# zju3dv/neuralbody

Measured on AMD Instinct MI355X. Metric: ray_samples_per_sec, higher is better.
Workload: dtype f16+f6/f4

## Files before the change

### neuralbody_amd/csrc/nb_march_fold.hip

```cpp
#include "nb_f6_ops.h"
#include "nb_march_hooks.h"

using namespace nbm;

namespace {

#ifndef NB_FP4_TERMS
#define NB_FP4_TERMS 3
#endif
constexpr bool FP4_K[2] = {(NB_FP4_TERMS & 1) != 0, (NB_FP4_TERMS & 2) != 0};
constexpr bool ANY_FP4 = FP4_K[0] || FP4_K[1];
constexpr int TERM_ORDER[2] = {(FP4_K[0] && !FP4_K[1]) ? 1 : 0, (FP4_K[0] && !FP4_K[1]) ? 0 : 1};
__host__ __device__ constexpr int term_pieces(int k) { return FP4_K[k] ? 1 : 2; }
__host__ __device__ constexpr int block_pieces(int mt) { return (4 * mt + mt * term_pieces(0) + mt * term_pieces(1) + 1) & ~1; }
__host__ __device__ constexpr int cross_piece(int mt, int slot, int m) {
    return 4 * mt + (slot == 0 ? 0 : mt * term_pieces(TERM_ORDER[0])) + m * term_pieces(TERM_ORDER[slot]);
}
constexpr int S_R = 8;
__host__ __device__ constexpr int phase_pieces(int nb, int mt) { return nb * block_pieces(mt); }
constexpr int N_PH = 4;
constexpr int PH_NB[N_PH] = {4, 4, 4, 2};
constexpr int PH_MT[N_PH] = {2, 2, 1, 1};
__host__ __device__ constexpr int phase_p0(int ph) {
    int p = 0;
// ... 365 lines not shown
    xhi = red_max16i(xhi); yhi = red_max16i(yhi); zhi = red_max16i(zhi);
    const int any = __builtin_amdgcn_ballot_w64(take) != 0ull;
    if (write && os == 0) {
        i32x4 *d = reinterpret_cast<i32x4 *>(actz + WBOX_OFF + (wslot * 4 + part) * 32);
        d[0] = i32x4{xlo, ylo, zlo, xhi};
        d[1] = i32x4{yhi, zhi, any, 0};
    }
}

struct Prep {
    int xlo, ylo, zlo, nx, nxy, n, k0;
    int K;
    int tier;
    int any;
};
__device__ __forceinline__ int box_count(int xlo, int ylo, int zlo, int xhi, int yhi, int zhi) {
    return (xhi < xlo || yhi < ylo || zhi < zlo) ? 0 : (xhi - xlo + 1) * (yhi - ylo + 1) * (zhi - zlo + 1);
}
template <int NW>
__device__ __forceinline__ Prep prep_wg(const char *actz, int part) {
    int xlo = BOX_BIG, ylo = BOX_BIG, zlo = BOX_BIG, xhi = -1, yhi = -1, zhi = -1;
    int n16[NW], any = 0;
#pragma unroll
    for (int w = 0; w < NW; ++w) {
        const i32x4 *s = reinterpret_cast<const i32x4 *>(actz + WBOX_OFF + (w * 4 + part) * 32);
        const i32x4 a = s[0], b = s[1];
        any |= b.z;
        n16[w] = box_count(a.x, a.y, a.z, a.w, b.x, b.y);
        xlo = min(xlo, a.x); ylo = min(ylo, a.y); zlo = min(zlo, a.z);
        xhi = max(xhi, a.w); yhi = max(yhi, b.x); zhi = max(zhi, b.y);
    }
    Prep p;
    p.xlo = xlo; p.ylo = ylo; p.zlo = zlo;
    p.nx = xhi - xlo + 1;
    p.nxy = p.nx * (yhi - ylo + 1);
    p.n = box_count(xlo, ylo, zlo, xhi, yhi, zhi);
    const int n0 = __builtin_amdgcn_readlane(p.n, 0), n1 = __builtin_amdgcn_readlane(p.n, 16), n2 = __builtin_amdgcn_readlane(p.n, 32),
              n3 = __builtin_amdgcn_readlane(p.n, 48);
    p.K = n0 + n1 + n2 + n3;
    p.k0 = part == 0 ? 0 : (part == 1 ? n0 : (part == 2 ? n0 + n1 : n0 + n1 + n2));
    p.tier = 0;
    p.any = any;
    if constexpr (NW > 1) {
        if (p.K > K_CAP && p.K <= KM_CAP) {
            p.tier = 3;
        } else if (p.K > K_CAP) {
            int worst = 0;
#pragma unroll
            for (int w = 0; w < NW; ++w)
                worst = max(worst, __builtin_amdgcn_readlane(n16[w], 0) + __builtin_amdgcn_readlane(n16[w], 16) +
                                       __builtin_amdgcn_readlane(n16[w], 32) + __builtin_amdgcn_readlane(n16[w], 48));
            p.tier = worst <= K_CAP ? 1 : 2;
        }
    }
    return p;
}

struct TblLoad {
    int rid[2], idx[2];
};
__device__ __forceinline__ TblLoad tbl_issue(const Prep &p, const Lvl &lv, int wave, int os) {
    TblLoad t;
    const float rcp_xy = __builtin_amdgcn_rcpf((float)max(p.nxy, 1)), rcp_x = __builtin_amdgcn_rcpf((float)max(p.nx, 1));
#pragma unroll
    for (int q = 0; q < 2; ++q) {
        const int j = 64 * q + 16 * wave + os;
        t.rid[q] = -1;
        t.idx[q] = -1;
        if (j < p.n) {
            const int vz = (int)(((float)j + 0.5f) * rcp_xy);
            const int r = mad24(vz, -p.nxy, j);
            const int vy = (int)(((float)r + 0.5f) * rcp_x);
            const int vx = mad24(vy, -p.nx, r);
            const int lin = mad24(mad24(p.zlo + vz, lv.H, p.ylo + vy), lv.W, p.xlo + vx);
            t.rid[q] = lv.grid[lin];
            t.idx[q] = p.k0 + j;
        }
    }
    return t;
}
__device__ __forceinline__ void tbl_store(char *actz, const TblLoad &t, const Lvl &lv, unsigned zero_off, int K, int tid) {
    unsigned *tbl = reinterpret_cast<unsigned *>(actz + TBL_OFF);
#pragma unroll
    for (int q = 0; q < 2; ++q)
        if (t.idx[q] >= 0) tbl[t.idx[q]] = t.rid[q] < 0 ? zero_off : (unsigned)(lv.rbase + t.rid[q]) << 10;
    if (tid < 16 && K + tid < ((K + 15) & ~15)) tbl[K + tid] = zero_off;
}
__device__ __forceinline__ void tbl_pass(char *actz, unsigned zero_off, int k_lo, int K, int tid) {
    if (tid >= K_CAP) return;
    unsigned *tbl = reinterpret_cast<unsigned *>(actz + TBL_OFF);
    const int k = k_lo + tid;
    unsigned e = zero_off;
    if (k < K) {
        const int k1 = *reinterpret_cast<const int *>(actz + LVL_OFF + 1 * 32 + 20), k2 = *reinterpret_cast<const int *>(actz + LVL_OFF + 2 * 32 + 20),
                  k3 = *reinterpret_cast<const int *>(actz + LVL_OFF + 3 * 32 + 20);
        const int L = (k >= k1) + (k >= k2) + (k >= k3);
        const i32x4 *lp = reinterpret_cast<const i32x4 *>(actz + LVL_OFF + L * 32);
        const i32x4 b0 = lp[0], b1 = lp[1];
        const Lvl lv = load_lvl(actz, L);
        const int j = k - b1.y;
        const float rcp_xy = __builtin_amdgcn_rcpf((float)max(b1.x, 1)), rcp_x = __builtin_amdgcn_rcpf((float)max(b0.w, 1));
        const int vz = (int)(((float)j + 0.5f) * rcp_xy);
        const int r = mad24(vz, -b1.x, j);
        const int vy = (int)(((float)r + 0.5f) * rcp_x);
        const int vx = mad24(vy, -b0.w, r);
        const int lin = mad24(mad24(b0.z + vz, lv.H, b0.y + vy), lv.W, b0.x + vx);
        const int rid = lv.grid[lin];
        if (rid >= 0) e = (unsigned)(lv.rbase + rid) << 10;
    }
    tbl[tid] = e;
}
__device__ __forceinline__ void lvl_store(char *actz, const Prep &p, int tid, int os, int part) {
    if (tid < 64 && os == 0) {
        i32x4 *d = reinterpret_cast<i32x4 *>(actz + LVL_OFF + part * 32);
        d[0] = i32x4{p.xlo, p.ylo, p.zlo, p.nx};
        d[1] = i32x4{p.nxy, p.k0, p.n, 0};
    }
    if (tid == 0) *reinterpret_cast<int *>(actz + HDR_OFF) = p.K;
}

struct UCfg {
    int nch, R;
    unsigned ring;
    int ring_off;
};
__device__ __forceinline__ UCfg ucfg_k(int K, unsigned lds_base, int wave);
__device__ __forceinline__ UCfg ucfg(const char *actz, unsigned lds_base, int wave) {
    return ucfg_k(__builtin_amdgcn_readfirstlane(*reinterpret_cast<const int *>(actz + HDR_OFF)), lds_base, wave);
}
__device__ __forceinline__ UCfg ucfg_k(int K, unsigned lds_base, int wave) {
    UCfg u;
    u.nch = (K + 15) >> 4;
    u.R = u.nch <= 3 ? u.nch : (u.nch == 4 ? 3 : 2);
    u.ring_off = WT_CHUNK * u.nch + wave * u.R * U_CHUNK;
    u.ring = lds_base + (unsigned)u.ring_off;
    return u;
}
__device__ __forceinline__ void dma_chunk(const MarchArgs &a, const char *actz, int lane, int wave, int c, unsigned dst) {
    const int v = ((lane >> 4) << 2) | ((lane >> 1) & 3);
    const unsigned e = *reinterpret_cast<const unsigned *>(actz + TBL_OFF + (16 * c + v) * 4);
    const unsigned voff0 = e + (unsigned)(64 * wave + 16 * ((lane >> 3) & 1) + 8 * (lane & 1)) * 2u;
    const char *base = a.fold.urows;
#pragma unroll
    for (int form = 0; form < 2; ++form)
#pragma unroll
        for (int m = 0; m < 2; ++m) {
            const unsigned voff = voff0 + form * 512 + m * 64;
            const unsigned d = dst + form * 2048 + m * 1024;
            asm volatile(
                "s_mov_b32 m0, %2\n\t"
                "s_nop 0\n\t"
                "global_load_lds_dwordx4 %0, %1"
                :
                : "v"(voff), "s"(base), "s"(d)
                : "memory", "m0");
        }
}
__device__ __forceinline__ void dma_initial(const MarchArgs &a, const char *actz, int lane, int wave, const UCfg &u) {
    for (int c = 0; c < u.R; ++c) dma_chunk(a, actz, lane, wave, c, u.ring + c * U_CHUNK);
}
__device__ __forceinline__ void dma_wait() { asm volatile("s_waitcnt vmcnt(0)" ::: "memory"); }

__device__ __forceinline__ void wt_build(char *actz, const Lvl &lv, const GridCoord &g, bool take, int wave, int os, int part, int nch,
                                         int k_lo = 0) {
    const int nt = wave >> 1, n = 16 * (wave & 1) + os;
    {
        char *z = actz + (part >> 1) * 2048 + nt * 1024 + ((part & 1) * 32 + n) * 16;
        for (int c = 0; c < nch; ++c) *reinterpret_cast<i32x4 *>(z + c * WT_CHUNK) = i32x4{0, 0, 0, 0};
    }
    if (take) {
        const i32x4 *lp = reinterpret_cast<const i32x4 *>(actz + LVL_OFF + part * 32);
        const i32x4 b0 = lp[0], b1 = lp[1];
        const LvlIdx q = level_index(lv, g);
        const float fx = (float)q.x0, fy = (float)q.y0, fz = (float)q.z0;
        const float wx[2] = {(fx + 1.f) - q.ix, q.ix - fx};
        const float wy[2] = {(fy + 1.f) - q.iy, q.iy - fy};
        const float wz[2] = {(fz + 1.f) - q.iz, q.iz - fz};
        const int kbase = b1.y - k_lo + mad24(q.z0 - b0.z, b1.x, mad24(q.y0 - b0.y, b0.w, q.x0 - b0.x));
        const int sbase = nt * 1024 + n * 16;
        float cw[8];
        int ad[8];
#pragma unroll
        for (int corner = 0; corner < 8; ++corner) {
            const int dx = corner & 1, dy = (corner >> 1) & 1, dz = corner >> 2;
            const int xx = q.x0 + dx, yy = q.y0 + dy, zz = q.z0 + dz;
            const bool inb = (unsigned)xx < (unsigned)lv.W && (unsigned)yy < (unsigned)lv.H && (unsigned)zz < (unsigned)lv.D;
            cw[corner] = (wx[dx] * wy[dy]) * wz[dz];
            const int k = kbase + dx + dy * b0.w + dz * b1.x;
            const int off = ((k << 8) & ~0xfff) | ((k << 6) & 0x200) | ((k << 1) & 0xe);
            ad[corner] = (inb && (unsigned)k < (unsigned)(16 * nch)) ? off + sbase : DUMMY_OFF;
        }
#pragma unroll
        for (int cp = 0; cp < 4; ++cp) {
            const unsigned h = cvt_pk_f16(cw[2 * cp], cw[2 * cp + 1]);
            const unsigned l = cvt_pk_f16(rem16<0>(cw[2 * cp], h), rem16<1>(cw[2 * cp + 1], h));
            *reinterpret_cast<unsigned short *>(actz + ad[2 * cp]) = (unsigned short)(h & 0xffffu);
            *reinterpret_cast<unsigned short *>(actz + ad[2 * cp + 1]) = (unsigned short)(h >> 16);
            *reinterpret_cast<unsigned short *>(actz + ad[2 * cp] + 2048) = (unsigned short)(l & 0xffffu);
            *reinterpret_cast<unsigned short *>(actz + ad[2 * cp + 1] + 2048) = (unsigned short)(l >> 16);
        }
    }
}

__device__ __forceinline__ f16x8 tr_frag(const char *p) {
    const s4v a = __builtin_amdgcn_ds_read_tr16_b64_v4i16((lds_s4p)(p));
    const s4v b = __builtin_amdgcn_ds_read_tr16_b64_v4i16((lds_s4p)(p + 256));
    typedef short s8v __attribute__((ext_vector_type(8)));
    return __builtin_bit_cast(f16x8, s8v{a[0], a[1], a[2], a[3], b[0], b[1], b[2], b[3]});
}
struct FoldFrags {
    f16x8 ah[2], al[2];
    i32x4 bh[2], bl[2];
};
__device__ __forceinline__ void fold_wait(int younger) {
    if (younger >= 2) asm volatile("s_waitcnt vmcnt(8)" ::: "memory");
    else if (younger == 1) asm volatile("s_waitcnt vmcnt(4)" ::: "memory");
    else asm volatile("s_waitcnt vmcnt(0)" ::: "memory");
}
__device__ __forceinline__ void fold_read(FoldFrags &f, const char *ub, const char *wtc) {
#pragma unroll
    for (int m = 0; m < 2; ++m) {
        f.ah[m] = tr_frag(ub + m * 1024);
        f.al[m] = tr_frag(ub + 2048 + m * 1024);
    }
#pragma unroll
    for (int n = 0; n < 2; ++n) {
        f.bh[n] = *reinterpret_cast<const i32x4 *>(wtc + n * 1024);
        f.bl[n] = *reinterpret_cast<const i32x4 *>(wtc + 2048 + n * 1024);
    }
}
__device__ __forceinline__ void fold_mma(const FoldFrags &f, f32x16 (&acc)[2][2]) {
#pragma unroll
    for (int p = 0; p < 3; ++p)
#pragma unroll
        for (int m = 0; m < 2; ++m)
#pragma unroll
            for (int n = 0; n < 2; ++n)
                acc[m][n] = __builtin_amdgcn_mfma_f32_32x32x16_f16(p == 2 ? f.al[m] : f.ah[m], __builtin_bit_cast(f16x8, p == 1 ? f.bl[n] : f.bh[n]),
                                                                   acc[m][n], 0, 0, 0);
}
__device__ __forceinline__ void fold_mfma(const MarchArgs &a, char *actz, int lane, int wave, const UCfg &u, f32x16 (&acc)[2][2],
                                          unsigned *tbuf = nullptr) {
    if (u.nch == 0) return;
    FOLD_SUB(17);
    const int l15 = lane & 15, g4 = lane >> 4;
    const int tro = (g4 >> 1) * 512 + (g4 & 1) * 128 + (l15 >> 2) * 32 + (l15 & 3) * 8;
    const char *wt = actz + lane * 16;
    const char *ring = actz + u.ring_off + tro;
    int issued = u.R - 1;
    FoldFrags f0, f1;
    fold_wait(issued);
    FOLD_SUB(18);
    fold_read(f0, ring, wt);
    NB_HOOK_FOLD_FIRST_READ(f0);
    FOLD_SUB(19);
    auto step = [&](FoldFrags &cur, FoldFrags &nxt, int c, int slot) {
        if (c + u.R < u.nch) {
            asm volatile("s_waitcnt lgkmcnt(0)" : "+v"(cur.ah[0]), "+v"(cur.ah[1]), "+v"(cur.al[0]), "+v"(cur.al[1])::"memory");
            dma_chunk(a, actz, lane, wave, c + u.R, u.ring + slot * U_CHUNK);
            issued = c + u.R;
        }
        if (c + 1 < u.nch) {
            const int ns = slot + 1 == u.R ? 0 : slot + 1;
            fold_wait(issued - (c + 1));
            fold_read(nxt, ring + ns * U_CHUNK, wt + (c + 1) * WT_CHUNK);
        }
        fold_mma(cur, acc);
    };
    int slot = 0;
    for (int c = 0; c < u.nch; c += 2) {
        step(f0, f1, c, slot);
        slot = slot + 1 == u.R ? 0 : slot + 1;
        if (c + 1 < u.nch) {
            step(f1, f0, c + 1, slot);
            slot = slot + 1 == u.R ? 0 : slot + 1;
        }
    }
#pragma unroll
    for (int m = 0; m < 2; ++m) asm volatile("" : "+v"(acc[m][0]), "+v"(acc[m][1]));
    FOLD_SUB(20);
    if (tbuf && lane == 0) tbuf[21] = (unsigned)u.nch;
}

struct WeightStore4 {
    float q[4] = {0.f, 0.f, 0.f, 0.f};
    __device__ __forceinline__ void push(const MarchArgs &a, long long ray, int s, int S, int part, bool valid, float w) {
        if ((S & 15) != 0) {
            if (valid && part == 0) a.weights[ray * S + s] = w;
            return;
        }
        const int slot = s & 15;
#pragma unroll
        for (int i = 0; i < 4; ++i)
            if (slot == part * 4 + i) q[i] = w;
        if (slot == 15 && valid)
            *reinterpret_cast<f32x4 *>(a.weights + ray * S + (s - 15) + part * 4) = f32x4{q[0], q[1], q[2], q[3]};
    }
};

__device__ __forceinline__ float head_sum(const char *actz, int off, float bias) {
    const f32x4 p = *reinterpret_cast<const f32x4 *>(actz + off);
    return ((p.x + p.y) + (p.z + p.w)) + bias;
}
__device__ __noinline__ void list_ill_ray(const char *actz, const float *pk, float *ill, int cap, int sample, int part, float z_step, int ray) {
    const float *recf = reinterpret_cast<const float *>(actz + RAY_OFF) + sample * RAY_FLOATS;
    const f32x4 c0 = *reinterpret_cast<const f32x4 *>(recf + 12);
    const float sigma_raw = head_sum(actz, SCR_A + sample * 16, pk[P_AB]);
    const bool hit = ray >= 0 && fabsf(sigma_raw) < NB_ILL_SIGMA && c0.x > NB_ILL_T_MIN;
    if (__builtin_amdgcn_ballot_w64(hit) == 0ull) return;
    int slot = -1;
    if (hit && part == 0) slot = atomicAdd(reinterpret_cast<int *>(ill), 1);
    slot = __builtin_amdgcn_ds_bpermute((sample & 15) << 2, slot);
    if (!hit || slot >= cap) return;
    float *irec = ill + NB_ILL_HEADER_FLOATS + (long long)slot * NB_ILL_RECORD_FLOATS;
    if (part == 0) {
        *reinterpret_cast<f32x4 *>(irec) = f32x4{__int_as_float(ray), c0.x, recf[16], recf[17]};
        *reinterpret_cast<f32x4 *>(irec + 4) = f32x4{z_step, __fmul_rn(1e10f, recf[11]), sigma_raw, 0.f};
    } else {
        const int ch = part - 1;
        irec[8 + ch] = part == 1 ? c0.y : (part == 2 ? c0.z : c0.w);
        irec[12 + ch] = head_sum(actz, SCR_C + (ch * 64 + sample) * 16, pk[P_RB + ch]);
    }
}

__device__ __forceinline__ void composite_step(char *actz, const float *pk, int sample, int part, float z_step, float z_after, bool last,
                                               const MarchArgs &a, long long ray, int sidx, int S, bool valid, WeightStore4 &wstore, bool ins) {
    float *recf = reinterpret_cast<float *>(actz + RAY_OFF) + sample * RAY_FLOATS;
    const f32x4 c0 = *reinterpret_cast<const f32x4 *>(recf + 12);
    const float sigma_raw = ins ? head_sum(actz, SCR_A + sample * 16, pk[P_AB]) : 0.f;
    const float d = last ? 1e10f : __fsub_rn(z_after, z_step);
    const float dist = __fmul_rn(d, recf[11]);
    const float sig = fmaxf(sigma_raw, 0.f);
    const float alpha = 1.f - expf(-sig * dist);
    const float w = alpha * c0.x;
    if (part == 0) {
        const float depth = recf[16], accw = recf[17];
        recf[12] = c0.x * (__fadd_rn(__fsub_rn(1.f, alpha), 1e-10f));
        recf[16] = fmaf(w, z_step, depth);
        recf[17] = accw + w;
    } else {
        const int ch = part - 1;
        const float o = ins ? head_sum(actz, SCR_C + (ch * 64 + sample) * 16, pk[P_RB + ch]) : 0.f;
        const float col = part == 1 ? c0.y : (part == 2 ? c0.z : c0.w);
        recf[12 + part] = fmaf(w, 1.f / (1.f + expf(-o)), col);
    }
    wstore.push(a, ray, sidx, S, part, valid, w);
    if (NB_HOOK_RAW_IS_OUTPUT && a.raw && valid && part == 0) {
        float o3[3];
#pragma unroll
        for (int ch = 0; ch < 3; ++ch) o3[ch] = ins ? head_sum(actz, SCR_C + (ch * 64 + sample) * 16, pk[P_RB + ch]) : 0.f;
        *reinterpret_cast<f32x4 *>(a.raw + (ray * S + sidx) * 4) = f32x4{o3[0], o3[1], o3[2], sigma_raw};
    }
}

__host__ __device__ inline int pe_slot_col(int a, int slot) {
    if (a >= 3 || slot >= 30) return -1;
    if (slot == 0) return 256 + 27 + a;
    if (slot <= 20) {
        const int k = (slot - 1) >> 1, is_cos = (slot - 1) & 1;
        return 256 + 27 + 3 + 6 * k + 3 * is_cos + a;
    }
    if (slot == 21) return 256 + a;
    const int k = (slot - 22) >> 1, is_cos = (slot - 22) & 1;
    return 256 + 3 + 6 * k + 3 * is_cos + a;
}

template <int MODE, bool CULL>
__global__ __launch_bounds__(256, 2) void nb_march_fold_kernel(MarchArgs a, const char *stream) {
    constexpr bool POINTS = MODE != 0, DENSITY_ONLY = MODE == 2;
    static_assert(!(CULL && POINTS), "sample culling is a property of the ray march");
    saturate_fp16_conversions();
    __shared__ __attribute__((aligned(16))) char lds[LDS_BYTES];
    char *act = lds;
    const int tid = threadIdx.x;
    const int lane = threadIdx.x & 63, wave = __builtin_amdgcn_readfirstlane(threadIdx.x >> 6);
    const int grp = xcd_remap(blockIdx.x, a.n_wave_groups);
    long long ray = (long long)grp * 64 + 16 * wave + (lane & 15);
    const long long n_units = POINTS ? a.n_pts : a.n_rays;
    bool valid = ray < n_units;
    if (!valid) ray = n_units - 1;
    if (!POINTS && a.ray_order) {
        if (a.ray_order[(long long)grp * 64] == NB_SLOT_DEAD) return;
        const int v = a.ray_order[(long long)grp * 64 + 16 * wave + (lane & 15)];
        valid = v >= 0;
        ray = valid ? v : -(long long)v - 1;
    }
    const int S = POINTS ? 1 : a.n_samples;
    {
        float ox, oy, oz, dx, dy, dz, near, far, dn, vx, vy, vz;
        if constexpr (POINTS) {
            ox = a.wpts[ray * 3 + 0], oy = a.wpts[ray * 3 + 1], oz = a.wpts[ray * 3 + 2];
            dx = DENSITY_ONLY ? 0.f : a.viewdir[ray * 3 + 0], dy = DENSITY_ONLY ? 0.f : a.viewdir[ray * 3 + 1];
            dz = DENSITY_ONLY ? 1.f : a.viewdir[ray * 3 + 2];
            near = far = 0.f;
            dn = 1.f;
            vx = dx, vy = dy, vz = dz;
        } else {
            ox = a.ray_o[ray * 3 + 0], oy = a.ray_o[ray * 3 + 1], oz = a.ray_o[ray * 3 + 2];
            dx = a.ray_d[ray * 3 + 0], dy = a.ray_d[ray * 3 + 1], dz = a.ray_d[ray * 3 + 2];
            near = a.near[ray], far = a.far[ray];
            dn = sqrtf(__fadd_rn(__fadd_rn(__fmul_rn(dx, dx), __fmul_rn(dy, dy)), __fmul_rn(dz, dz)));
            vx = dx / dn, vy = dy / dn, vz = dz / dn;
        }
        if ((lane >> 4) == 0) {
            f32x4 *rec = reinterpret_cast<f32x4 *>(lds + RAY_OFF) + (16 * wave + (lane & 15)) * (RAY_FLOATS / 4);
            rec[0] = f32x4{ox, oy, oz, near};
            rec[1] = f32x4{dx, dy, dz, far};
            rec[2] = f32x4{vx, vy, vz, dn};
            rec[3] = f32x4{1.f, 0.f, 0.f, 0.f};
            rec[4] = f32x4{0.f, 0.f, 0.f, 0.f};
        }
    }
    const float *tr = (!POINTS && a.t_rand) ? a.t_rand + ray * S : nullptr;
    auto tval = [&](int s) -> float { return ((cfloat_ptr)a.t_vals)[s]; };
    auto z_at = [&](int s, float near, float far) -> float {
        if constexpr (POINTS) return 0.f;
        const float zc = z_lin(near, far, tval(s));
        if (!tr) return zc;
        const float lower = s == 0 ? zc : 0.5f * __fadd_rn(zc, z_lin(near, far, tval(s - 1)));
        const float upper = s == S - 1 ? zc : 0.5f * __fadd_rn(z_lin(near, far, tval(s + 1)), zc);
        return __fadd_rn(lower, __fmul_rn(__fsub_rn(upper, lower), tr[s]));
    };

    {
        float *prm = reinterpret_cast<float *>(lds + PRM_OFF);
        for (int i = tid; i < P_SIZE; i += 256) {
            float v;
            if (i < P_B1) v = a.pk[F_OFF_B0 + i - P_B0];
            else if (i < P_B2) v = a.pk[F_OFF_B1 + i - P_B1];
            else if (i < P_AW) v = a.pk[F_OFF_B2 + i - P_B2];
            else if (i < P_RW) v = a.pk[F_OFF_AW + i - P_AW];
            else if (i < P_AB) v = a.pk[F_OFF_RW + i - P_RW];
            else if (i < P_RB) v = a.pk[F_OFF_AB + i - P_AB];
            else if (i < P_LB) v = a.pk[F_OFF_RB + i - P_RB];
            else v = DENSITY_ONLY ? 0.f : a.lb[256 + i - P_LB];
            prm[i] = v;
        }
        if (tid < 4) {
            int *lc = reinterpret_cast<int *>(lds + LC_OFF + tid * 48);
            const unsigned long long gp = (unsigned long long)a.fold.grid[tid];
            lc[0] = a.sc.dhw[tid][0]; lc[1] = a.sc.dhw[tid][1]; lc[2] = a.sc.dhw[tid][2];
            lc[3] = __float_as_int(a.sc.fm1[tid][2]); lc[4] = __float_as_int(a.sc.fm1[tid][1]); lc[5] = __float_as_int(a.sc.fm1[tid][0]);
            lc[6] = __float_as_int(a.sc.fp1[tid][2]); lc[7] = __float_as_int(a.sc.fp1[tid][1]); lc[8] = __float_as_int(a.sc.fp1[tid][0]);
            lc[9] = (int)(unsigned)(gp & 0xffffffffull); lc[10] = (int)(unsigned)(gp >> 32);
            lc[11] = a.fold.row_base[tid];
        }
        __syncthreads();
    }
    const __amdgpu_buffer_rsrc_t wrsrc =
        __builtin_amdgcn_make_buffer_rsrc(const_cast<char *>(stream) + (size_t)wave * WAVE_STREAM, 0, WAVE_STREAM, 0x00020000);
    WRing ring;
    WeightStore4 wstore;
    typedef void __attribute__((address_space(3))) *lptr_t;
    const unsigned lds_base = (unsigned)(unsigned long long)(lptr_t)(lds);

    float z_cur;
    GridCoord g;
    bool ins = true;
    int tier, active;
    auto prep_sequential = [&](int sn, float &z_out, int lane_c) {
        const int os = lane_c & 15, part = lane_c >> 4, sample = 16 * wave + os;
        const f32x4 *rec = reinterpret_cast<const f32x4 *>(lds + RAY_OFF) + sample * (RAY_FLOATS / 4);
        const f32x4 ro = rec[0], rd = rec[1];
        z_out = z_at(sn, ro.w, rd.w);
        const float px = __fadd_rn(ro.x, __fmul_rn(rd.x, z_out)), py = __fadd_rn(ro.y, __fmul_rn(rd.y, z_out)),
                    pz = __fadd_rn(ro.z, __fmul_rn(rd.z, z_out));
        g = grid_coords(a.sc, px, py, pz);
        if constexpr (CULL) ins = cull_inside(a.cull, a.sc, px, py, pz);
        const Lvl lv = load_lvl(lds, part);
        prep_boxes(lds, lv, g, ins, wave, true, os, part);
        __syncthreads();
        const Prep pr = prep_wg<4>(lds, part);
        tier = __builtin_amdgcn_readfirstlane(pr.tier);
        active = __builtin_amdgcn_readfirstlane(pr.any);
        if (tier == 0) {
            const TblLoad tl = tbl_issue(pr, lv, wave, os);
            tbl_store(lds, tl, lv, a.fold.zero_off, pr.K, tid);
        }
        lvl_store(lds, pr, tid, os, part);
    };
    auto fetch_and_weights = [&](int lane_c) {
        if (tier == 0 && active) {
            const int os = lane_c & 15, part = lane_c >> 4;
            const UCfg u = ucfg(lds, lds_base, wave);
            dma_initial(a, lds, lane_c, wave, u);
            const Lvl lv = load_lvl(lds, part);
            wt_build(lds, lv, g, ins, wave, os, part, u.nch);
        }
    };
    prep_sequential(0, z_cur, lane);
    __syncthreads();
    fetch_and_weights(lane);
    for (int s = 0; s < S; ++s) {
        int zero = 0, lane_i = lane;
        asm volatile("" : "+s"(zero), "+v"(lane_i));
        const int hi = lane_i >> 5, os = lane_i & 15, part = lane_i >> 4, sample = 16 * wave + os;
        const WSrc wl = {wrsrc, (unsigned)lane_i * 16u};
        char *actz = act + zero;
        const float *pk = reinterpret_cast<const float *>(actz + PRM_OFF);
        const f32x4 *rec = reinterpret_cast<const f32x4 *>(actz + RAY_OFF) + sample * (RAY_FLOATS / 4);
        const int sn = sample >> 5, ss = sample & 31;
        const bool more = s + 1 < S;
        const bool ins_cur = ins;
        float z_next = 0.f;
        int tier_next = 0, active_next = 1;
        NB_HOOK_STEP_BEGIN;
        FOLD_STAMP(0);
        __syncthreads();
        FOLD_STAMP(1);
        if (!CULL || active) {
            f32x16 acc[2][2];
            init_bias<2>(pk + P_B0, 2 * wave, hi, acc);
            if (tier == 0) {
                const UCfg u = ucfg(actz, lds_base, wave);
                fold_mfma(a, actz, lane_i, wave, u, acc, NB_HOOK_TBUF);
            } else if (tier == 3) {
                const Lvl lv = load_lvl(actz, part);
                const int K = __builtin_amdgcn_readfirstlane(*reinterpret_cast<const int *>(actz + HDR_OFF));
                for (int k_lo = 0; k_lo < K; k_lo += K_CAP) {
                    tbl_pass(actz, a.fold.zero_off, k_lo, K, tid);
                    __syncthreads();
                    const UCfg u = ucfg_k(min(K - k_lo, K_CAP), lds_base, wave);
                    dma_initial(a, actz, lane_i, wave, u);
                    wt_build(actz, lv, g, ins_cur, wave, os, part, u.nch, k_lo);
                    __syncthreads();
                    fold_mfma(a, actz, lane_i, wave, u, acc);
                    __syncthreads();
                }
            } else {
                const Lvl lv = load_lvl(actz, part);
                const int n_groups = tier == 1 ? 4 : 64;
                for (int gi = 0; gi < n_groups; ++gi) {
                    const bool take = ins_cur && (tier == 1 ? wave == gi : sample == gi);
                    prep_boxes(actz, lv, g, take, 0, wave == (tier == 1 ? gi : gi >> 4), os, part);
                    __syncthreads();
                    const Prep pr = prep_wg<1>(actz, part);
                    const TblLoad tl = tbl_issue(pr, lv, wave, os);
                    tbl_store(actz, tl, lv, a.fold.zero_off, pr.K, tid);
                    lvl_store(actz, pr, tid, os, part);
                    __syncthreads();
                    const UCfg u = ucfg(actz, lds_base, wave);
                    dma_initial(a, actz, lane_i, wave, u);
                    wt_build(actz, lv, g, take, wave, os, part, u.nch);
                    __syncthreads();
                    fold_mfma(a, actz, lane_i, wave, u, acc);
                    __syncthreads();
                }
            }
            FOLD_DUMP(0, 2)
            FOLD_STAMP(2);
            ring_prime<P_L1>(wl, ring);
            publish_s(actz, lane_i, wave, acc);
            FOLD_STAMP(3);
            init_bias<2>(pk + P_B1, 2 * wave, hi, acc);
            Conv6 pec;
            {
                const f32x4 ro = rec[0], rd = rec[1], rv = rec[2];
                const float xa = part == 0 ? __fadd_rn(ro.x, __fmul_rn(rd.x, z_cur))
                                           : (part == 1 ? __fadd_rn(ro.y, __fmul_rn(rd.y, z_cur)) : __fadd_rn(ro.z, __fmul_rn(rd.z, z_cur)));
                const float va = part == 0 ? rv.x : (part == 1 ? rv.y : rv.z);
                Rev2 tx, tv;
                float e[32];
                auto pe_fill = [&](auto tc) {
                    constexpr int t = decltype(tc)::value;
                    if constexpr (t == 0) {
                        tx = rev2(xa);
                        tv = rev2(va);
                        e[0] = xa;
                        e[21] = va;
                        e[30] = 0.f;
                        e[31] = 0.f;
                    } else if constexpr (t <= 10) {
                        sincos_rev2<t - 1>(tx, e[2 * t - 1], e[2 * t]);
                    } else if constexpr (t <= 14) {
                        sincos_rev2<t - 11>(tv, e[2 * t], e[2 * t + 1]);
                    } else if constexpr (t >= 16) {
                        constexpr int i = t - 16;
                        conv6_pair<2 * i>(pec, e[4 * i], e[4 * i + 1]);
                        conv6_pair<2 * i + 1>(pec, e[4 * i + 2], e[4 * i + 3]);
                    }
                };
                if constexpr (DENSITY_ONLY) layer_s<P_L1, 2, 4, true>(wl, actz, lane_i, ring, acc);
                else layer_s<P_L1, 2, 4, true>(wl, actz, lane_i, ring, acc, pe_fill);
            }
            HalfBlock peh;
            if constexpr (!DENSITY_ONLY) peh = conv6_finish(pec);
            FOLD_DUMP(1, 2)
            FOLD_STAMP(4);
            publish_s(actz, lane_i, wave, acc);
            FOLD_STAMP(5);
            init_bias<2>(pk + P_B2, 2 * wave, hi, acc);
            layer_s<P_L2, 2, 4, true>(wl, actz, lane_i, ring, acc);
            FOLD_DUMP(2, 2)
            FOLD_STAMP(6);
            if (more) {
                const f32x4 ro = rec[0], rd = rec[1];
                z_next = z_at(s + 1, ro.w, rd.w);
                const float px = __fadd_rn(ro.x, __fmul_rn(rd.x, z_next)), py = __fadd_rn(ro.y, __fmul_rn(rd.y, z_next)),
                            pz = __fadd_rn(ro.z, __fmul_rn(rd.z, z_next));
                g = grid_coords(a.sc, px, py, pz);
                if constexpr (CULL) ins = cull_inside(a.cull, a.sc, px, py, pz);
                const Lvl lv = load_lvl(actz, part);
                prep_boxes(actz, lv, g, ins, wave, true, os, part);
            }
            FOLD_STAMP(7);
            if constexpr (DENSITY_ONLY) {
#pragma unroll
                for (int m = 0; m < 2; ++m)
#pragma unroll
                    for (int n = 0; n < 2; ++n)
#pragma unroll
                        for (int r = 0; r < 16; ++r) acc[m][n][r] = relu1(acc[m][n][r]);
            } else {
                publish_s(actz, lane_i, wave, acc);
            }
            FOLD_STAMP(8);
            {
#pragma unroll
                for (int n = 0; n < 2; ++n) {
                    float s4[4] = {0.f, 0.f, 0.f, 0.f};
#pragma unroll
                    for (int m = 0; m < 2; ++m) {
                        const f32x4 *aw = reinterpret_cast<const f32x4 *>(pk + P_AW + hi * 128 + 16 * (2 * wave + m));
#pragma unroll
                        for (int q4 = 0; q4 < 4; ++q4) {
                            const f32x4 w4 = aw[q4];
                            s4[0] = fmaf(w4.x, acc[m][n][4 * q4 + 0], s4[0]);
                            s4[1] = fmaf(w4.y, acc[m][n][4 * q4 + 1], s4[1]);
                            s4[2] = fmaf(w4.z, acc[m][n][4 * q4 + 2], s4[2]);
                            s4[3] = fmaf(w4.w, acc[m][n][4 * q4 + 3], s4[3]);
                        }
                    }
                    float sa = add_halves((s4[0] + s4[1]) + (s4[2] + s4[3]));
                    if (hi == 0) reinterpret_cast<float *>(actz + SCR_A)[(n * 32 + (lane_i & 31)) * 4 + wave] = sa;
                }
            }
            if constexpr (!DENSITY_ONLY) {
                TblLoad tl;
                int k_next = 0;
                if (more) {
                    const Lvl lv = load_lvl(actz, part);
                    const Prep pr = prep_wg<4>(actz, part);
                    tier_next = __builtin_amdgcn_readfirstlane(pr.tier);
                    active_next = __builtin_amdgcn_readfirstlane(pr.any);
                    k_next = __builtin_amdgcn_readfirstlane(pr.K);
                    tl.rid[0] = tl.rid[1] = tl.idx[0] = tl.idx[1] = -1;
                    if (tier_next == 0) tl = tbl_issue(pr, lv, wave, os);
                    lvl_store(actz, pr, tid, os, part);
                }
                FOLD_STAMP(9);
                init_bias<1>(pk + P_LB, wave, hi, acc);
                layer_s<P_VG, 1, 4, false>(wl, actz, lane_i, ring, acc);
                FOLD_STAMP(10);
                if (more && tier_next == 0) {
                    const Lvl lv = load_lvl(actz, part);
                    tbl_store(actz, tl, lv, a.fold.zero_off, k_next, tid);
                }
                __syncthreads();
                ring_prime<P_VP>(wl, ring);
                store_halfblock(actz, part >> 1, part & 1, sn, ss, peh);
                __syncthreads();
                FOLD_STAMP(11);
                layer_s<P_VP, 1, 2, false>(wl, actz, lane_i, ring, acc);
                FOLD_STAMP(12);
                FOLD_DUMP(3, 1)
                {
#pragma unroll
                    for (int n = 0; n < 2; ++n) {
                        float rl[16];
#pragma unroll
                        for (int r = 0; r < 16; ++r) rl[r] = relu1(acc[0][n][r]);
#pragma unroll
                        for (int ch = 0; ch < 3; ++ch) {
                            const f32x4 *rw = reinterpret_cast<const f32x4 *>(pk + P_RW + (ch * 2 + hi) * 64 + 16 * wave);
                            float c4[4] = {0.f, 0.f, 0.f, 0.f};
#pragma unroll
                            for (int q4 = 0; q4 < 4; ++q4) {
                                const f32x4 w4 = rw[q4];
                                c4[0] = fmaf(w4.x, rl[4 * q4 + 0], c4[0]);
                                c4[1] = fmaf(w4.y, rl[4 * q4 + 1], c4[1]);
                                c4[2] = fmaf(w4.z, rl[4 * q4 + 2], c4[2]);
                                c4[3] = fmaf(w4.w, rl[4 * q4 + 3], c4[3]);
                            }
                            float sc = add_halves((c4[0] + c4[1]) + (c4[2] + c4[3]));
                            if (hi == 0) reinterpret_cast<float *>(actz + SCR_C)[(ch * 64 + n * 32 + (lane_i & 31)) * 4 + wave] = sc;
                        }
                    }
                }
            }
        } else if (more) {
            prep_sequential(s + 1, z_next, lane_i);
            tier_next = tier;
            active_next = active;
        }
        FOLD_STAMP(13);
        __syncthreads();
        FOLD_STAMP(14);
        if (more) {
            tier = tier_next;
            active = active_next;
            fetch_and_weights(lane_i);
        }
        FOLD_STAMP(15);
        {
            if constexpr (POINTS) {
                if (valid && part == 0) {
                    const float sigma = head_sum(actz, SCR_A + sample * 16, pk[P_AB]);
                    if constexpr (DENSITY_ONLY) {
                        a.raw_out[ray] = sigma;
                    } else {
                        float o3[3];
#pragma unroll
                        for (int ch = 0; ch < 3; ++ch) o3[ch] = head_sum(actz, SCR_C + (ch * 64 + sample) * 16, pk[P_RB + ch]);
                        *reinterpret_cast<f32x4 *>(a.raw_out + ray * 4) = f32x4{o3[0], o3[1], o3[2], sigma};
                    }
                }
            } else {
                if (s + 1 >= S && a.ill != nullptr)
                    list_ill_ray(actz, pk, a.ill, a.ill_cap, sample, part, z_cur, (valid && (!CULL || ins_cur)) ? (int)ray : -1);
                composite_step(actz, pk, sample, part, z_cur, z_next, s + 1 >= S, a, ray, s, S, valid, wstore, !CULL || ins_cur);
            }
        }
        FOLD_STAMP(16);
        z_cur = z_next;
    }
    if (!POINTS && valid && (lane >> 4) == 0) {
        const f32x4 *rec = reinterpret_cast<const f32x4 *>(lds + RAY_OFF) + (16 * wave + (lane & 15)) * (RAY_FLOATS / 4);
        const f32x4 c0 = rec[3], c1 = rec[4];
        RayAccum ra;
        ra.T = c0.x; ra.cr = c0.y; ra.cg = c0.z; ra.cb = c0.w; ra.depth = c1.x; ra.accw = c1.y;
        ra.store(a, ray);
    }
}

__device__ __forceinline__ int frag_bias_index(int f) {
    const int t = f >> 5, i = f & 31;
    return (t * 2 + ((i >> 2) & 1)) * 16 + (i & 3) + 4 * (i >> 3);
}
__device__ __forceinline__ double frag_row_dot(const float *wfrag, const float *h, int row) {
    const f32x4 *w4 = reinterpret_cast<const f32x4 *>(wfrag) + (size_t)(row >> 5) * 32 * 64 + (row & 31);
    double s = 0.0;
    for (int g = 0; g < 32; ++g)
#pragma unroll
        for (int hi = 0; hi < 2; ++hi) {
            const f32x4 w = w4[g * 64 + hi * 32];
            const float *hh = h + 8 * g + 4 * hi;
            s = fma((double)w.x, (double)hh[0], s);
            s = fma((double)w.y, (double)hh[1], s);
            s = fma((double)w.z, (double)hh[2], s);
            s = fma((double)w.w, (double)hh[3], s);
        }
    return s;
}
__global__ __launch_bounds__(256) void nb_march_fixup_kernel(MarchArgs a) {
    __shared__ float rec[NB_ILL_RECORD_FLOATS];
    __shared__ float cw[32];
    __shared__ int crow[32];
    __shared__ float h[2][256];
    __shared__ double red[4];
    const int tid = threadIdx.x;
    int *hdr = reinterpret_cast<int *>(a.ill);
    const int n = min(hdr[0], a.ill_cap);
    const int S = a.n_samples;
    for (int it = blockIdx.x; it < n; it += gridDim.x) {
        __syncthreads();
        if (tid < NB_ILL_RECORD_FLOATS) rec[tid] = a.ill[NB_ILL_HEADER_FLOATS + (long long)it * NB_ILL_RECORD_FLOATS + tid];
        __syncthreads();
        const long long ray = __float_as_int(rec[0]);
        const float z = rec[4];
        if (tid < 32) {
            const int L = tid >> 3, corner = tid & 7;
            const float px = __fadd_rn(a.ray_o[ray * 3 + 0], __fmul_rn(a.ray_d[ray * 3 + 0], z)),
                        py = __fadd_rn(a.ray_o[ray * 3 + 1], __fmul_rn(a.ray_d[ray * 3 + 1], z)),
                        pz = __fadd_rn(a.ray_o[ray * 3 + 2], __fmul_rn(a.ray_d[ray * 3 + 2], z));
            const GridCoord g = grid_coords(a.sc, px, py, pz);
            Lvl lv;
            lv.D = a.sc.dhw[L][0]; lv.H = a.sc.dhw[L][1]; lv.W = a.sc.dhw[L][2];
            lv.fmx = a.sc.fm1[L][2]; lv.fmy = a.sc.fm1[L][1]; lv.fmz = a.sc.fm1[L][0];
            lv.fpx = a.sc.fp1[L][2]; lv.fpy = a.sc.fp1[L][1]; lv.fpz = a.sc.fp1[L][0];
            const LvlIdx q = level_index(lv, g);
            const float fx = (float)q.x0, fy = (float)q.y0, fz = (float)q.z0;
            const int dx = corner & 1, dy = (corner >> 1) & 1, dz = corner >> 2;
            const float wx = dx ? q.ix - fx : (fx + 1.f) - q.ix, wy = dy ? q.iy - fy : (fy + 1.f) - q.iy, wz = dz ? q.iz - fz : (fz + 1.f) - q.iz;
            const int xx = q.x0 + dx, yy = q.y0 + dy, zz = q.z0 + dz;
            const bool inb = (unsigned)xx < (unsigned)lv.W && (unsigned)yy < (unsigned)lv.H && (unsigned)zz < (unsigned)lv.D;
            int row = -1;
            if (inb) {
                const int rid = a.fold.grid[L][((size_t)zz * lv.H + yy) * lv.W + xx];
                if (rid >= 0) row = a.fold.row_base[L] + rid;
            }
            cw[tid] = (wx * wy) * wz;
            crow[tid] = row;
        }
        __syncthreads();
        {
            double s = (double)a.pk[F_OFF_B0 + frag_bias_index(tid)];
            for (int c = 0; c < 32; ++c) {
                if (crow[c] < 0) continue;
                const _Float16 *u = reinterpret_cast<const _Float16 *>(a.fold.urows) + (size_t)crow[c] * 512;
                s = fma((double)cw[c], (double)(float)u[tid] + (double)(float)u[256 + tid], s);
            }
            h[0][tid] = fmaxf((float)s, 0.f);
        }
        __syncthreads();
        h[1][tid] = fmaxf((float)((double)a.pk[F_OFF_B1 + frag_bias_index(tid)] + frag_row_dot(a.pk + F_OFF_B0 + 256, h[0], tid)), 0.f);
        __syncthreads();
        const float h3 = fmaxf((float)((double)a.pk[F_OFF_B2 + frag_bias_index(tid)] + frag_row_dot(a.pk + F_OFF_B1 + 256, h[1], tid)), 0.f);
        {
            const int t = tid >> 5, i = tid & 31;
            double p = (double)a.pk[F_OFF_AW + ((i >> 2) & 1) * 128 + 16 * t + (i & 3) + 4 * (i >> 3)] * (double)h3;
#pragma unroll
            for (int m = 32; m >= 1; m >>= 1) p += __shfl_xor(p, m);
            if ((tid & 63) == 0) red[tid >> 6] = p;
        }
        __syncthreads();
        if (tid == 0) {
            const float sigma = (float)(((red[0] + red[1]) + (red[2] + red[3])) + (double)a.pk[F_OFF_AB]);
            RayAccum ra;
            ra.T = rec[1]; ra.depth = rec[2]; ra.accw = rec[3];
            ra.cr = rec[8]; ra.cg = rec[9]; ra.cb = rec[10];
            const float out4[4] = {rec[12], rec[13], rec[14], sigma};
            const float w = ra.add(out4, z, rec[5]);
            ra.store(a, ray);
            a.weights[ray * S + (S - 1)] = w;
            if (a.raw) a.raw[(ray * S + (S - 1)) * 4 + 3] = sigma;
            if ((sigma > 0.f) != (rec[6] > 0.f)) atomicAdd(&hdr[1], 1);
        }
    }
}

__device__ __forceinline__ int phase_col(int ph, int b, int kh, int e) {
    if (ph < 3) return col_hidden(32 * b + e, kh);
    return pe_slot_col(2 * b + kh, e);
}
__device__ __forceinline__ float phase_weight(const nb_mlp_params &p, const float *f32_blob, int ph, int row, int b, int kh, int e) {
    const int col = phase_col(ph, b, kh, e);
    if (col < 0) return 0.f;
    if (ph == 0) return p.fc1_w[row * 256 + col];
    if (ph == 1) return p.fc2_w[row * 256 + col];
    if (ph == 2) {
        const int tt = col >> 5, rr = col & 31, hi2 = (rr >> 2) & 1, r2 = (rr & 3) + 4 * (rr >> 3), q2 = 16 * tt + r2;
        double s = 0.0;
        for (int m = 0; m < 256; ++m)
            s += (double)p.view_w[row * 346 + m] *
                 (double)f32_blob[F_OFF_L4 + (((m >> 5) * 32 + (q2 >> 2)) * 64 + (hi2 * 32 + (m & 31))) * 4 + (q2 & 3)];
        return (float)s;
    }
    return p.view_w[row * 346 + col];
}

__device__ __forceinline__ unsigned fp4_e2m1_bits(float v) {
    const unsigned sgn = v < 0.f ? 8u : 0u;
    const float a = fminf(fabsf(v), 6.f);
    constexpr float grid[8] = {0.f, 0.5f, 1.f, 1.5f, 2.f, 3.f, 4.f, 6.f};
    unsigned code = 0;
    float best = a;
    for (unsigned c = 1; c < 8; ++c) {
        const float d = fabsf(a - grid[c]);
        if (d < best || (d == best && (c & 1u) == 0u)) {
            best = d;
            code = c;
        }
    }
    return sgn | code;
}

__global__ void nb_pack_fold_kernel(nb_mlp_params p, const float *__restrict__ f32_blob, unsigned *__restrict__ out, int *__restrict__ stats) {
    const int t = blockIdx.x * blockDim.x + threadIdx.x;
    if (t >= 4 * P_TOTAL * 64) return;
    const int lane = t & 63, piece = (t >> 6) % P_TOTAL, w = (t >> 6) / P_TOTAL;
    const int i = lane & 31, kg = lane >> 5;
    int ph = 0, p0 = 0;
    for (int q = 0; q < N_PH; ++q) {
        const int n = phase_pieces(PH_NB[q], PH_MT[q]);
        if (piece < p0 + n) {
            ph = q;
            break;
        }
        p0 += n;
    }
    const int mt = PH_MT[ph], ppb = block_pieces(mt);
    const int rel = piece - p0, b = rel / ppb, r = rel % ppb;
    unsigned w32[4] = {0u, 0u, 0u, 0u};
    if (r < 4 * mt) {
        const int j = r / mt, m = r % mt;
        const int row = (mt == 2 ? 64 * w + 32 * m : 32 * w) + i;
        for (int q = 0; q < 8; q += 2) {
            const f16x2 hp = {(_Float16)phase_weight(p, f32_blob, ph, row, b, kg, 8 * j + q),
                              (_Float16)phase_weight(p, f32_blob, ph, row, b, kg, 8 * j + q + 1)};
            w32[q / 2] = __builtin_bit_cast(unsigned, hp);
        }
    } else {
        int r6 = r - 4 * mt, k = -1, m = 0, half = 0;
        for (int slot = 0; slot < 2; ++slot) {
            const int kk = TERM_ORDER[slot], width = mt * term_pieces(kk);
            if (r6 < width) {
                k = kk;
                m = r6 / term_pieces(kk);
                half = r6 % term_pieces(kk);
                break;
            }
            r6 -= width;
        }
        if (k >= 0) {
            const bool four = FP4_K[k];
            const float top = four ? 6.f : 7.5f;
            const int row = (mt == 2 ? 64 * w + 32 * m : 32 * w) + i;
            float wv[32], amax = 0.f;
            for (int e = 0; e < 32; ++e) {
                const int n = k ? e : 16 * (e & 1) + (e >> 1);
                const float wt = phase_weight(p, f32_blob, ph, row, b, kg, n);
                const float h = (float)(_Float16)wt;
                wv[e] = k ? wt - h : h;
                amax = fmaxf(amax, fabsf(wv[e]));
            }
            int ex = 0;
            if (amax > 0.f && amax < 3.0e38f) {
                ex = ilogbf(amax / top);
                if (ldexpf(top, ex) < amax) ++ex;
                ex = min(max(ex, -120), 120);
            }
            if (four) {
                for (int e = 0; e < 32; ++e) w32[e >> 3] |= fp4_e2m1_bits(ldexpf(wv[e], -ex)) << (4 * (e & 7));
                unsigned char *sc = reinterpret_cast<unsigned char *>(out) + (size_t)w * WAVE_STREAM + (size_t)P_TOTAL * 1024 +
                                    (size_t)(phase_s0(ph) + b) * 256 + lane * 4 + (k * mt + m);
                *sc = (unsigned char)(127 + ex);
            } else {
                unsigned w8[8] = {0u, 0u, 0u, 0u, 0u, 0u, 0u, 0u};
                for (int e = 0; e < 32; ++e) {
                    const unsigned code = fp6_e2m3_bits(ldexpf(wv[e], -ex));
                    const int bit = 6 * e;
                    w8[bit >> 5] |= code << (bit & 31);
                    if ((bit & 31) > 26) w8[(bit >> 5) + 1] |= code >> (32 - (bit & 31));
                }
                w8[6] = (unsigned)(127 + ex);
                for (int q = 0; q < 4; ++q) w32[q] = w8[4 * half + q];
            }
            if (k == 0 && half == 0) {
                int small = 0, nz = 0;
                for (int e = 0; e < 32; ++e) {
                    nz += wv[e] != 0.f;
                    small += wv[e] != 0.f && fabsf(wv[e]) < 0.125f * amax;
                }
                const int layer = ph < 2 ? ph : 2;
                atomicAdd(&stats[2 * layer], small);
                atomicAdd(&stats[2 * layer + 1], nz);
            }
        }
    }
    unsigned *dst = reinterpret_cast<unsigned *>(reinterpret_cast<char *>(out) + (size_t)w * WAVE_STREAM) + ((size_t)piece * 64 + lane) * 4;
    for (int q = 0; q < 4; ++q) dst[q] = w32[q];
}

}

namespace nbm {

long long fold_stream_floats() { return (long long)4 * WAVE_STREAM / 4 + 8; }

int pack_fold_stream(const nb_mlp_params *p, float *packed, long long stream_off, hipStream_t st) {
    const long long n = (long long)4 * P_TOTAL * 64;
    int *stats = reinterpret_cast<int *>(packed + stream_off + (long long)4 * WAVE_STREAM / 4);
    NB_REQUIRE(hipMemsetAsync(stats, 0, 8 * sizeof(int), st) == hipSuccess, "pack_fold_stream: hipMemsetAsync failed");
    hipLaunchKernelGGL(nb_pack_fold_kernel, dim3(nb_ceil_div(n, 256)), dim3(256), 0, st, *p, packed,
                       reinterpret_cast<unsigned *>(packed + stream_off), stats);
    NB_CHECK_LAUNCH("nb_pack_fold_kernel");
    return NB_OK;
}

int launch_march_fold(MarchArgs a, long long stream_off, hipStream_t st) {
    a.n_wave_groups = (int)nb_ceil_div(a.ray_order ? a.n_slots : a.n_rays, 64);
    const char *stream = reinterpret_cast<const char *>(a.pk + stream_off);
    if (a.ill) NB_REQUIRE(hipMemsetAsync(a.ill, 0, NB_ILL_HEADER_FLOATS * sizeof(float), st) == hipSuccess, "nb_march: hipMemsetAsync(ill_scratch) failed");
    if (a.cull.n_views) hipLaunchKernelGGL((nb_march_fold_kernel<0, true>), dim3(a.n_wave_groups), dim3(256), 0, st, a, stream);
    else hipLaunchKernelGGL((nb_march_fold_kernel<0, false>), dim3(a.n_wave_groups), dim3(256), 0, st, a, stream);
    NB_CHECK_LAUNCH("nb_march_fold_kernel");
    if (a.ill) {
        hipLaunchKernelGGL(nb_march_fixup_kernel, dim3(NB_ILL_FIXUP_BLOCKS), dim3(256), 0, st, a);
        NB_CHECK_LAUNCH("nb_march_fixup_kernel");
    }
    return NB_OK;
}

int launch_points_fold(MarchArgs a, int density_only, long long stream_off, hipStream_t st) {
    a.n_wave_groups = (int)nb_ceil_div(a.n_pts, 64);
    const char *stream = reinterpret_cast<const char *>(a.pk + stream_off);
    if (density_only) hipLaunchKernelGGL((nb_march_fold_kernel<2, false>), dim3(a.n_wave_groups), dim3(256), 0, st, a, stream);
    else hipLaunchKernelGGL((nb_march_fold_kernel<1, false>), dim3(a.n_wave_groups), dim3(256), 0, st, a, stream);
    NB_CHECK_LAUNCH("nb_march_fold_kernel (points)");
    return NB_OK;
}

}
```

Measured before the change: 1.410 billion.

## Move positional-encoding fill into view layer and rematerialize per-iteration values

Moves the positional-encoding sin/cos fill and conv6 packing from the first layer to the later view-direction layer, so the half-block is built just before it is stored. This shortens its live range across the density layers. Also recomputes tid, ray and t_rand pointers inside the loop behind an asm barrier, reloads level data instead of holding it, and force-inlines list_ill_ray, all to cut register pressure and call overhead. The risk is that the fill now overlaps a smaller layer and hides less latency, and that the extra reloads add LDS traffic.

```diff
diff --git a/neuralbody_amd/csrc/nb_march_fold.hip b/neuralbody_amd/csrc/nb_march_fold.hip
--- a/neuralbody_amd/csrc/nb_march_fold.hip
+++ b/neuralbody_amd/csrc/nb_march_fold.hip
@@ -691,7 +691,7 @@
     const f32x4 p = *reinterpret_cast<const f32x4 *>(actz + off);
     return ((p.x + p.y) + (p.z + p.w)) + bias;
 }
-__device__ __noinline__ void list_ill_ray(const char *actz, const float *pk, float *ill, int cap, int sample, int part, float z_step, int ray) {
+__device__ __forceinline__ void list_ill_ray(const char *actz, const float *pk, float *ill, int cap, int sample, int part, float z_step, int ray) {
     const float *recf = reinterpret_cast<const float *>(actz + RAY_OFF) + sample * RAY_FLOATS;
     const f32x4 c0 = *reinterpret_cast<const f32x4 *>(recf + 12);
     const float sigma_raw = head_sum(actz, SCR_A + sample * 16, pk[P_AB]);
@@ -800,7 +800,8 @@
             rec[4] = f32x4{0.f, 0.f, 0.f, 0.f};
         }
     }
-    const float *tr = (!POINTS && a.t_rand) ? a.t_rand + ray * S : nullptr;
+    const float *tr_c = (!POINTS && a.t_rand) ? a.t_rand + ray * S : nullptr;
+    const float *tr = tr_c;
     auto tval = [&](int s) -> float { return ((cfloat_ptr)a.t_vals)[s]; };
     auto z_at = [&](int s, float near, float far) -> float {
         if constexpr (POINTS) return 0.f;
@@ -848,6 +849,7 @@
     bool ins = true;
     int tier, active;
     auto prep_sequential = [&](int sn, float &z_out, int lane_c) {
+        const int tid_c = wave * 64 + lane_c;
         const int os = lane_c & 15, part = lane_c >> 4, sample = 16 * wave + os;
         const f32x4 *rec = reinterpret_cast<const f32x4 *>(lds + RAY_OFF) + sample * (RAY_FLOATS / 4);
         const f32x4 ro = rec[0], rd = rec[1];
@@ -864,9 +866,9 @@
         active = __builtin_amdgcn_readfirstlane(pr.any);
         if (tier == 0) {
             const TblLoad tl = tbl_issue(pr, lv, wave, os);
-            tbl_store(lds, tl, lv, a.fold.zero_off, pr.K, tid);
-        }
-        lvl_store(lds, pr, tid, os, part);
+            tbl_store(lds, tl, lv, a.fold.zero_off, pr.K, tid_c);
+        }
+        lvl_store(lds, pr, tid_c, os, part);
     };
     auto fetch_and_weights = [&](int lane_c) {
         if (tier == 0 && active) {
@@ -880,9 +882,13 @@
     prep_sequential(0, z_cur, lane);
     __syncthreads();
     fetch_and_weights(lane);
+    int lane_i = lane;
+    long long ray_i = ray;
     for (int s = 0; s < S; ++s) {
-        int zero = 0, lane_i = lane;
-        asm volatile("" : "+s"(zero), "+v"(lane_i));
+        int zero = 0;
+        asm volatile("" : "+s"(zero), "+v"(lane_i), "+v"(ray_i));
+        const int tid_i = wave * 64 + lane_i;
+        if (!POINTS && a.t_rand) tr = a.t_rand + ray_i * S;
         const int hi = lane_i >> 5, os = lane_i & 15, part = lane_i >> 4, sample = 16 * wave + os;
         const WSrc wl = {wrsrc, (unsigned)lane_i * 16u};
         char *actz = act + zero;
@@ -904,33 +910,31 @@
                 const UCfg u = ucfg(actz, lds_base, wave);
                 fold_mfma(a, actz, lane_i, wave, u, acc, NB_HOOK_TBUF);
             } else if (tier == 3) {
-                const Lvl lv = load_lvl(actz, part);
                 const int K = __builtin_amdgcn_readfirstlane(*reinterpret_cast<const int *>(actz + HDR_OFF));
                 for (int k_lo = 0; k_lo < K; k_lo += K_CAP) {
-                    tbl_pass(actz, a.fold.zero_off, k_lo, K, tid);
+                    tbl_pass(actz, a.fold.zero_off, k_lo, K, tid_i);
                     __syncthreads();
                     const UCfg u = ucfg_k(min(K - k_lo, K_CAP), lds_base, wave);
                     dma_initial(a, actz, lane_i, wave, u);
-                    wt_build(actz, lv, g, ins_cur, wave, os, part, u.nch, k_lo);
+                    wt_build(actz, load_lvl(actz, part), g, ins_cur, wave, os, part, u.nch, k_lo);
                     __syncthreads();
                     fold_mfma(a, actz, lane_i, wave, u, acc);
                     __syncthreads();
                 }
             } else {
-                const Lvl lv = load_lvl(actz, part);
                 const int n_groups = tier == 1 ? 4 : 64;
                 for (int gi = 0; gi < n_groups; ++gi) {
                     const bool take = ins_cur && (tier == 1 ? wave == gi : sample == gi);
-                    prep_boxes(actz, lv, g, take, 0, wave == (tier == 1 ? gi : gi >> 4), os, part);
+                    prep_boxes(actz, load_lvl(actz, part), g, take, 0, wave == (tier == 1 ? gi : gi >> 4), os, part);
                     __syncthreads();
                     const Prep pr = prep_wg<1>(actz, part);
-                    const TblLoad tl = tbl_issue(pr, lv, wave, os);
-                    tbl_store(actz, tl, lv, a.fold.zero_off, pr.K, tid);
-                    lvl_store(actz, pr, tid, os, part);
+                    const TblLoad tl = tbl_issue(pr, load_lvl(actz, part), wave, os);
+                    tbl_store(actz, tl, load_lvl(actz, part), a.fold.zero_off, pr.K, tid_i);
+                    lvl_store(actz, pr, tid_i, os, part);
                     __syncthreads();
                     const UCfg u = ucfg(actz, lds_base, wave);
                     dma_initial(a, actz, lane_i, wave, u);
-                    wt_build(actz, lv, g, take, wave, os, part, u.nch);
+                    wt_build(actz, load_lvl(actz, part), g, take, wave, os, part, u.nch);
                     __syncthreads();
                     fold_mfma(a, actz, lane_i, wave, u, acc);
                     __syncthreads();
@@ -942,38 +946,7 @@
             publish_s(actz, lane_i, wave, acc);
             FOLD_STAMP(3);
             init_bias<2>(pk + P_B1, 2 * wave, hi, acc);
-            Conv6 pec;
-            {
-                const f32x4 ro = rec[0], rd = rec[1], rv = rec[2];
-                const float xa = part == 0 ? __fadd_rn(ro.x, __fmul_rn(rd.x, z_cur))
-                                           : (part == 1 ? __fadd_rn(ro.y, __fmul_rn(rd.y, z_cur)) : __fadd_rn(ro.z, __fmul_rn(rd.z, z_cur)));
-                const float va = part == 0 ? rv.x : (part == 1 ? rv.y : rv.z);
-                Rev2 tx, tv;
-                float e[32];
-                auto pe_fill = [&](auto tc) {
-                    constexpr int t = decltype(tc)::value;
-                    if constexpr (t == 0) {
-                        tx = rev2(xa);
-                        tv = rev2(va);
-                        e[0] = xa;
-                        e[21] = va;
-                        e[30] = 0.f;
-                        e[31] = 0.f;
-                    } else if constexpr (t <= 10) {
-                        sincos_rev2<t - 1>(tx, e[2 * t - 1], e[2 * t]);
-                    } else if constexpr (t <= 14) {
-                        sincos_rev2<t - 11>(tv, e[2 * t], e[2 * t + 1]);
-                    } else if constexpr (t >= 16) {
-                        constexpr int i = t - 16;
-                        conv6_pair<2 * i>(pec, e[4 * i], e[4 * i + 1]);
-                        conv6_pair<2 * i + 1>(pec, e[4 * i + 2], e[4 * i + 3]);
-                    }
-                };
-                if constexpr (DENSITY_ONLY) layer_s<P_L1, 2, 4, true>(wl, actz, lane_i, ring, acc);
-                else layer_s<P_L1, 2, 4, true>(wl, actz, lane_i, ring, acc, pe_fill);
-            }
-            HalfBlock peh;
-            if constexpr (!DENSITY_ONLY) peh = conv6_finish(pec);
+            layer_s<P_L1, 2, 4, true>(wl, actz, lane_i, ring, acc);
             FOLD_DUMP(1, 2)
             FOLD_STAMP(4);
             publish_s(actz, lane_i, wave, acc);
@@ -1035,15 +1008,45 @@
                     k_next = __builtin_amdgcn_readfirstlane(pr.K);
                     tl.rid[0] = tl.rid[1] = tl.idx[0] = tl.idx[1] = -1;
                     if (tier_next == 0) tl = tbl_issue(pr, lv, wave, os);
-                    lvl_store(actz, pr, tid, os, part);
+                    lvl_store(actz, pr, tid_i, os, part);
                 }
                 FOLD_STAMP(9);
                 init_bias<1>(pk + P_LB, wave, hi, acc);
-                layer_s<P_VG, 1, 4, false>(wl, actz, lane_i, ring, acc);
+                HalfBlock peh;
+                {
+                    Conv6 pec;
+                    const f32x4 ro = rec[0], rd = rec[1], rv = rec[2];
+                    const float xa = part == 0 ? __fadd_rn(ro.x, __fmul_rn(rd.x, z_cur))
+                                               : (part == 1 ? __fadd_rn(ro.y, __fmul_rn(rd.y, z_cur)) : __fadd_rn(ro.z, __fmul_rn(rd.z, z_cur)));
+                    const float va = part == 0 ? rv.x : (part == 1 ? rv.y : rv.z);
+                    Rev2 tx, tv;
+                    float e[32];
+                    auto pe_fill = [&](auto tc) {
+                        constexpr int t = decltype(tc)::value;
+                        if constexpr (t == 0) {
+                            tx = rev2(xa);
+                            tv = rev2(va);
+                            e[0] = xa;
+                            e[21] = va;
+                            e[30] = 0.f;
+                            e[31] = 0.f;
+                        } else if constexpr (t <= 10) {
+                            sincos_rev2<t - 1>(tx, e[2 * t - 1], e[2 * t]);
+                        } else if constexpr (t <= 14) {
+                            sincos_rev2<t - 11>(tv, e[2 * t], e[2 * t + 1]);
+                        } else if constexpr (t >= 16) {
+                            constexpr int i = t - 16;
+                            conv6_pair<2 * i>(pec, e[4 * i], e[4 * i + 1]);
+                            conv6_pair<2 * i + 1>(pec, e[4 * i + 2], e[4 * i + 3]);
+                        }
+                    };
+                    layer_s<P_VG, 1, 4, false>(wl, actz, lane_i, ring, acc, pe_fill);
+                    peh = conv6_finish(pec);
+                }
                 FOLD_STAMP(10);
                 if (more && tier_next == 0) {
                     const Lvl lv = load_lvl(actz, part);
-                    tbl_store(actz, tl, lv, a.fold.zero_off, k_next, tid);
+                    tbl_store(actz, tl, lv, a.fold.zero_off, k_next, tid_i);
                 }
                 __syncthreads();
                 ring_prime<P_VP>(wl, ring);
@@ -1096,29 +1099,29 @@
                 if (valid && part == 0) {
                     const float sigma = head_sum(actz, SCR_A + sample * 16, pk[P_AB]);
                     if constexpr (DENSITY_ONLY) {
-                        a.raw_out[ray] = sigma;
+                        a.raw_out[ray_i] = sigma;
                     } else {
                         float o3[3];
 #pragma unroll
                         for (int ch = 0; ch < 3; ++ch) o3[ch] = head_sum(actz, SCR_C + (ch * 64 + sample) * 16, pk[P_RB + ch]);
-                        *reinterpret_cast<f32x4 *>(a.raw_out + ray * 4) = f32x4{o3[0], o3[1], o3[2], sigma};
+                        *reinterpret_cast<f32x4 *>(a.raw_out + ray_i * 4) = f32x4{o3[0], o3[1], o3[2], sigma};
                     }
                 }
             } else {
                 if (s + 1 >= S && a.ill != nullptr)
-                    list_ill_ray(actz, pk, a.ill, a.ill_cap, sample, part, z_cur, (valid && (!CULL || ins_cur)) ? (int)ray : -1);
-                composite_step(actz, pk, sample, part, z_cur, z_next, s + 1 >= S, a, ray, s, S, valid, wstore, !CULL || ins_cur);
+                    list_ill_ray(actz, pk, a.ill, a.ill_cap, sample, part, z_cur, (valid && (!CULL || ins_cur)) ? (int)ray_i : -1);
+                composite_step(actz, pk, sample, part, z_cur, z_next, s + 1 >= S, a, ray_i, s, S, valid, wstore, !CULL || ins_cur);
             }
         }
         FOLD_STAMP(16);
         z_cur = z_next;
     }
-    if (!POINTS && valid && (lane >> 4) == 0) {
-        const f32x4 *rec = reinterpret_cast<const f32x4 *>(lds + RAY_OFF) + (16 * wave + (lane & 15)) * (RAY_FLOATS / 4);
+    if (!POINTS && valid && (lane_i >> 4) == 0) {
+        const f32x4 *rec = reinterpret_cast<const f32x4 *>(lds + RAY_OFF) + (16 * wave + (lane_i & 15)) * (RAY_FLOATS / 4);
         const f32x4 c0 = rec[3], c1 = rec[4];
         RayAccum ra;
         ra.T = c0.x; ra.cr = c0.y; ra.cg = c0.z; ra.cb = c0.w; ra.depth = c1.x; ra.accw = c1.y;
-        ra.store(a, ray);
+        ra.store(a, ray_i);
     }
 }
 
```

Measured after the change: 1.424 billion, median of 6. No clear change (+1.0%).
